# changhaonan/A3VLM

Hardware: AMD Instinct MI355X
Metric: image-text samples/sec (train) + articulation-decode tok/s (higher is better)
Workload: dtype bf16

## Files before the change

### a3vlm_amd/csrc/a3v_train.hip

```cpp
#include "a3v_common.h"

namespace {

template <typename T>
__global__ __launch_bounds__(256) void transpose_kernel(const T* __restrict__ src, int64_t lds_, int64_t bs_s,
                                                        T* __restrict__ dst, int64_t ldd, int64_t bs_d, int R, int C, int Rpad) {
  __shared__ T tile[64][64 + 2];
  const T* s = src + blockIdx.z * bs_s;
  T* d = dst + blockIdx.z * bs_d;
  const int r0 = blockIdx.y * 64, c0 = blockIdx.x * 64;
  const int tx = threadIdx.x & 63, ty = threadIdx.x >> 6;
  for (int i = ty; i < 64; i += 4) {
    const int r = r0 + i, c = c0 + tx;
    tile[i][tx] = (r < R && c < C) ? s[(int64_t)r * lds_ + c] : (T)0.f;
  }
  __syncthreads();
  for (int i = ty; i < 64; i += 4) {
    const int c = c0 + i, r = r0 + tx;
    if (c < C && r < Rpad) d[(int64_t)c * ldd + r] = tile[tx][i];
  }
}

__global__ __launch_bounds__(256) void transpose_bf16_vec_kernel(const bf16_t* __restrict__ src, int64_t lds_, int64_t bs_s,
                                                                 bf16_t* __restrict__ dst, int64_t ldd, int64_t bs_d, int R, int C, int Rpad,
// ... 1125 lines not shown
    if (t.d2) reinterpret_cast<bf16_t*>(t.d2)[r * t.s2r + c * t.s2c] = f2bf(pp);
  }
}
}

extern "C" int a3v_adamw_multi(const a3v_adamw_tensor* table_dev, int n_tensors, int64_t max_n, float lr, float beta1, float beta2, float eps,
                               float weight_decay, int64_t step, const float* grad_scale, void* stream) {
  if (!table_dev || n_tensors <= 0 || max_n <= 0 || step < 1) return A3V_ERR_ARG;
  if (n_tensors > 65535) return A3V_ERR_SHAPE;
  const double bc1 = 1.0 - pow((double)beta1, (double)step), bc2 = 1.0 - pow((double)beta2, (double)step);
  const float step_size = (float)((double)lr / bc1), inv_bc2_sqrt = (float)(1.0 / sqrt(bc2));
  const float decay = (float)(1.0 - (double)lr * (double)weight_decay);
  int64_t blocks = (max_n / 4 + 255) / 256;
  if (blocks > 64) blocks = 64;
  if (blocks < 1) blocks = 1;
  hipLaunchKernelGGL(adamw_multi_kernel, dim3((unsigned)blocks, (unsigned)n_tensors), dim3(256), 0, (hipStream_t)stream, table_dev, decay, beta1,
                     beta2, step_size, inv_bc2_sqrt, eps, grad_scale);
  A3V_LAUNCH_CHECK();
  return A3V_OK;
}

namespace {
__global__ __launch_bounds__(256) void lora_refresh_kernel(const float* __restrict__ wa, const float* __restrict__ wb, int r, int in_f, int nj,
                                                           bf16_t* __restrict__ A, int64_t lda, bf16_t* __restrict__ At, int64_t ldat,
                                                           bf16_t* __restrict__ B, int64_t ldb, bf16_t* __restrict__ Bt, int64_t ldbt,
                                                           int col0, int row0) {
  const int t = blockIdx.x * 256 + threadIdx.x;
  if (t < in_f) {
    for (int i = 0; i < r; ++i) {
      const bf16_t v = f2bf(wa[(int64_t)i * in_f + t]);
      A[(int64_t)(col0 + i) * lda + t] = v;
      At[(int64_t)t * ldat + col0 + i] = v;
    }
  }
  if (t < nj) {
    for (int i = 0; i < r; ++i) {
      const bf16_t v = f2bf(wb[(int64_t)t * r + i]);
      B[(int64_t)(row0 + t) * ldb + col0 + i] = v;
      Bt[(int64_t)(col0 + i) * ldbt + row0 + t] = v;
    }
  }
}
}

extern "C" int a3v_lora_refresh(const float* lora_a, const float* lora_b, int r, int in_f, int nj, void* A, int64_t lda, void* At,
                                int64_t ldat, void* B, int64_t ldb, void* Bt, int64_t ldbt, int col0, int row0, void* stream) {
  if (!lora_a || !lora_b || !A || !At || !B || !Bt || r <= 0 || in_f <= 0 || nj <= 0 || col0 < 0 || row0 < 0) return A3V_ERR_ARG;
  const int n = in_f > nj ? in_f : nj;
  hipLaunchKernelGGL(lora_refresh_kernel, dim3((n + 255) / 256), dim3(256), 0, ST, lora_a, lora_b, r, in_f, nj, (bf16_t*)A, lda, (bf16_t*)At, ldat,
                     (bf16_t*)B, ldb, (bf16_t*)Bt, ldbt, col0, row0);
  A3V_LAUNCH_CHECK();
  return A3V_OK;
}
```

### a3vlm_amd/lib.py

```python
from __future__ import annotations

import ctypes
import os
from ctypes import c_float, c_int, c_int64, c_void_p

_HERE = os.path.dirname(os.path.abspath(__file__))
LIB_PATH = os.environ.get("A3V_LIB_PATH") or os.path.join(_HERE, "liba3vlm_hip.so")

BF16, F32 = 0, 1
EPI_NONE, EPI_BIAS, EPI_GELU, EPI_QUICKGELU, EPI_RESIDUAL, EPI_SWIGLU, EPI_OUT_F32, EPI_RES_F32 = 0, 1, 2, 4, 8, 16, 32, 64
EPI_SWIGLU_BWD = 128

EPI_TILE_128, EPI_TILE_256, EPI_TILE_256PP = 1 << 16, 1 << 17, 1 << 18
EPI_TILE_192PP = 1 << 23

P, I, L, F = c_void_p, c_int, c_int64, c_float

SIGNATURES = {
    "a3v_version": (I, []),
    "a3v_reload_env": (I, []),
    "a3v_gemm_nt": (I, [P, L, P, L, P, L, I, I, I, P, P, L, I, I, P]),
    "a3v_gemm_qkv_rope": (I, [P, L, P, L, I, P, L, P, P, P, L, P, L, P, I, I, I, I, I, I, I, I, P]),
    "a3v_gemm_nt_fp8": (I, [P, L, P, P, L, P, P, L, I, I, I, P, P, L, I, P]),
    "a3v_gemm_qkv_rope_fp8": (I, [P, L, P, P, L, P, I, P, L, P, P, P, I, I, I, I, I, I, I, I, P]),
# ... 8 lines not shown
    "a3v_lora_gb_scatter": (I, [P, L, I, I, P, P, P, P]),
    "a3v_adamw_multi": (I, [P, I, L, F, F, F, F, F, L, P, P]),
    "a3v_scale_cast": (I, [P, I, P, I, L, F, P]),
    "a3v_sumsq_partials": (I, [P, L, P, P]),
    "a3v_grad_bucket_allreduce": (I, [P, P, L, P, I, P]),
    "a3v_grad_bucket_reduce_scatter": (I, [P, P, L, P, P, P, I, P]),
    "a3v_param_shard_all_gather": (I, [P, P, P, L, P]),
    "a3v_rccl_comm_count": (I, [P]),
    "a3v_rccl_available": (I, []),
    "a3v_gemm_nn": (I, [P, L, P, L, P, L, I, I, I, P, L, I, P]),
    "a3v_gemm_tn": (I, [P, L, P, L, P, L, I, I, I, P, L, I, P]),
    "a3v_gemm_tn_sumsq": (I, [P, L, P, L, P, L, I, I, I, P, L, I, P, L, P]),
    "a3v_gemm_tn_sumsq_slots": (L, [I, I]),
    "a3v_gemm_set_workspace": (I, [P, L]),
    "a3v_gemm_set_workspace_for": (I, [P, P, L]),
    "a3v_gemm_nt_splitk": (I, [P, L, P, L, P, I, I, I, I, P]),
    "a3v_splitk_reduce": (I, [P, I, I, I, P, L, I, I, P]),
    "a3v_gemm_skinny_split": (I, [I, I, I]),
    "a3v_gemm_skinny_ws_bytes": (L, [I, I, I]),
    "a3v_gemm_skinny_fp8": (I, [P, L, P, L, P, P, L, I, I, I, P, L, I, P, P]),
    "a3v_quantize_nf4_ws_bytes": (L, [I, I]),
    "a3v_quantize_nf4": (I, [P, I, I, P, P, P, P]),
    "a3v_dequantize_nf4": (I, [P, P, P, L, I, I, P]),
    "a3v_gemm_skinny_nf4": (I, [P, L, P, L, P, P, L, I, I, I, P, L, I, P, P]),
    "a3v_gemm_skinny": (I, [P, L, P, L, P, L, I, I, I, P, L, I, P, P]),
    "a3v_rmsnorm": (I, [P, L, P, P, L, I, I, F, I, I, I, P]),
    "a3v_layernorm": (I, [P, L, P, P, P, L, P, I, I, F, I, I, I, P]),
    "a3v_rope_kvcache": (I, [P, L, P, L, P, P, P, I, I, I, I, I, I, I, I, I, P]),
    "a3v_vt_pack": (I, [P, L, P, I, I, I, I, I, I, P]),
    "a3v_attention_scratch_floats": (L, [I, I, I, I]),
    "a3v_attention": (I, [P, P, P, P, I, I, I, I, I, I, ctypes.POINTER(c_int64), I, P, I, P]),
    "a3v_embed_assemble": (I, [P, L, P, P, I, I, I, I, I, I, I, P]),
    "a3v_fill_rows": (I, [P, P, L, P, I, I, I, I, P]),
    "a3v_patch_im2col": (I, [P, P, I, I, I, I, I, I, I, P]),
    "a3v_split_views": (I, [P, P, I, I, I, I, P]),
    "a3v_vit_embed": (I, [P, P, P, P, I, I, I, I, P]),
    "a3v_argmax": (I, [P, L, P, I, I, P]),
    "a3v_sample_top_p": (I, [P, L, I, I, F, F, P, P, P]),
    "a3v_preprocess_image": (I, [P, I, I, I, I, I, P, P, P, I, P, P, I, I, P, P, I, P, P, P]),
    "a3v_preprocess_batch": (I, [P, I, P, I, P, L, P, L, I, P, P, P]),
    "a3v_generate_step": (I, [P, L, P, I, I, P, L, P, L, I, P, P, I, P, P, P, P]),
    "a3v_count_valid": (I, [P, I, P, P]),
    "a3v_cross_entropy": (I, [P, L, P, P, P, L, P, F, I, I, I, P]),
    "a3v_attention_lse": (I, [P, P, P, P, P, I, I, I, I, I, I, ctypes.POINTER(c_int64), I, I, P]),
    "a3v_transpose": (I, [P, L, L, P, L, L, I, I, I, I, I, P]),
    "a3v_rmsnorm_bwd_scratch_floats": (L, [I, I]),
    "a3v_rmsnorm_bwd": (I, [P, L, P, P, L, P, L, P, P, I, I, F, I, P]),
    "a3v_rmsnorm_bwd_cast": (I, [P, L, P, P, L, P, L, P, P, I, I, F, I, P, L, P]),
    "a3v_rmsnorm_bwd_bf16": (I, [P, L, P, P, L, P, L, P, P, I, I, F, P]),
    "a3v_layernorm_bwd_bf16": (I, [P, L, P, P, L, P, P, L, P, P, I, I, F, P]),
    "a3v_embed_bwd_bf16": (I, [P, L, P, P, I, I, I, I, I, P]),
    "a3v_layernorm_bwd": (I, [P, L, P, P, L, P, P, L, P, P, I, I, F, I, P]),
    "a3v_swiglu_fwd": (I, [P, L, P, L, I, I, I, I, P]),
    "a3v_swiglu_bwd": (I, [P, L, P, L, P, L, I, I, I, I, P]),
    "a3v_cast": (I, [P, L, I, P, L, I, I, I, P]),
    "a3v_add2d": (I, [P, L, P, L, I, I, I, P]),
    "a3v_rope_bwd_pack": (I, [P, P, P, P, L, P, I, I, I, I, I, I, I, P]),
    "a3v_attention_bwd": (I, [P, P, L, L, P, L, L, L, P, P, P, P, P, P, P, P, I, I, I, I, I, I, I, P]),
    "a3v_attention_bwd_workspace_bytes": (L, [I, I, I, I, I]),
    "a3v_attention_bwd_mfma": (I, [P, P, L, L, P, L, L, L, P, P, P, P, P, P, P, I, I, I, I, I, I, P]),
    "a3v_embed_bwd": (I, [P, L, P, P, I, I, I, I, I, P]),
    "a3v_rows_sum": (I, [P, L, P, I, I, P, I, P]),
}

class LlamaLayer(ctypes.Structure):
    _fields_ = [(n, c_void_p) for n in ("attn_norm_w", "wqkv", "wo", "ffn_norm_w", "w13", "w2", "k_cache", "vt_cache",
                                        "wqkv_q", "wqkv_s", "wo_q", "wo_s", "w13_q", "w13_s", "w2_q", "w2_s",
                                        "wqkv_n4", "wqkv_n4s", "wo_n4", "wo_n4s", "w13_n4", "w13_n4s", "w2_n4", "w2_n4s")]


class ImageDesc(ctypes.Structure):
    _fields_ = [("src", c_void_p), ("coeffs", c_void_p), ("bounds", c_void_p), ("H", c_int), ("W", c_int), ("side", c_int), ("pad_x", c_int),
                ("pad_y", c_int), ("ksize", c_int)]


SIGNATURES["a3v_llama_decode_step"] = (I, [ctypes.POINTER(LlamaLayer), I, P, P, P, P, P, P, P, P, I, I, I, I, I, I, I, I, F, P])
SIGNATURES["a3v_llama_decode_step_form"] = (I, [I, I, I, I, I, I, I])

_lib = None


def load() -> ctypes.CDLL:
    global _lib
    if _lib is not None:
        return _lib
    if not os.path.isfile(LIB_PATH):
        raise RuntimeError(
            f"{LIB_PATH} not found: the HIP extension is not built. Run "
            "`python -c 'import __graft_entry__ as g; g.build()'` (or `make -C a3vlm_amd/csrc`). "
            "a3vlm_amd has no non-HIP fallback.")
    import torch
    lib = ctypes.CDLL(LIB_PATH)
    for name, (res, args) in SIGNATURES.items():
        fn = getattr(lib, name)
        fn.restype = res
        fn.argtypes = args
    _lib = lib
    return lib


class env:

    def __init__(self, **kw):
        self.kw = {k: str(v) for k, v in kw.items()}
        self.old = {}

# ... 28 lines not shown
```

### a3vlm_amd/ops.py

```python
from __future__ import annotations

import ctypes
from typing import Optional

import torch

from . import lib as _l
from .lib import BF16, F32, EPI_BIAS, EPI_GELU, EPI_QUICKGELU, EPI_RESIDUAL, EPI_SWIGLU, EPI_OUT_F32, EPI_RES_F32, EPI_SWIGLU_BWD

_DT = {torch.bfloat16: BF16, torch.float32: F32}


def dt(t: torch.Tensor) -> int:
    try:
        return _DT[t.dtype]
    except KeyError:
        raise TypeError(f"a3vlm_amd supports bf16/fp32 tensors, got {t.dtype}")


def _p(t: Optional[torch.Tensor]):
    return None if t is None else t.data_ptr()


def _stream() -> int:
# ... 433 lines not shown


_rb_scratch = {}


def rmsnorm_bwd(x, w, dy, dh, dw, eps, dh_lowp=None):
    _dev(x, w, dy, dh, dw, dh_lowp)
    assert w.dtype == torch.float32 and x.dtype == dh.dtype and x.dtype in (torch.float32, torch.bfloat16)
    rows, dim = x.shape
    scratch = None
    if dw is not None:
        need = int(_l.load().a3v_rmsnorm_bwd_scratch_floats(rows, dim))
        scratch = _rb_scratch.get(x.device)
        if scratch is None or scratch.numel() < need:
            scratch = torch.empty(need, dtype=torch.float32, device=x.device)
            _rb_scratch[x.device] = scratch
    if x.dtype == torch.bfloat16:
        assert dh_lowp is None and dy.dtype == torch.bfloat16
        rc = _l.load().a3v_rmsnorm_bwd_bf16(_p(x), x.stride(0), _p(w), _p(dy), dy.stride(0), _p(dh), dh.stride(0), _p(dw), _p(scratch), rows,
                                            dim, eps, _stream())
        _l.check(rc, "a3v_rmsnorm_bwd_bf16")
        return
    if dh_lowp is not None:
        assert dh_lowp.dtype == torch.bfloat16 and dh_lowp.shape == dh.shape
        rc = _l.load().a3v_rmsnorm_bwd_cast(_p(x), x.stride(0), _p(w), _p(dy), dy.stride(0), _p(dh), dh.stride(0), _p(dw), _p(scratch), rows,
                                            dim, eps, dt(dy), _p(dh_lowp), dh_lowp.stride(0), _stream())
        _l.check(rc, "a3v_rmsnorm_bwd_cast")
        return
    rc = _l.load().a3v_rmsnorm_bwd(_p(x), x.stride(0), _p(w), _p(dy), dy.stride(0), _p(dh), dh.stride(0), _p(dw), _p(scratch), rows, dim,
                                   eps, dt(dy), _stream())
    _l.check(rc, "a3v_rmsnorm_bwd")


def layernorm_bwd(x, w, dy, row_map, dx, dw, db, eps=1e-5):
    _dev(x, w, dy, row_map, dx, dw, db)
    rows, dim = x.shape
    if dy.dtype == torch.bfloat16:
        rc = _l.load().a3v_layernorm_bwd_bf16(_p(x), x.stride(0), _p(w), _p(dy), dy.stride(0), _p(row_map), _p(dx), dx.stride(0),
                                              _p(dw), _p(db), rows, dim, eps, _stream())
        _l.check(rc, "a3v_layernorm_bwd_bf16")
        return
    rc = _l.load().a3v_layernorm_bwd(_p(x), x.stride(0), _p(w), _p(dy), dy.stride(0), _p(row_map), _p(dx), dx.stride(0),
                                     _p(dw), _p(db), rows, dim, eps, dt(x), _stream())
    _l.check(rc, "a3v_layernorm_bwd")


def swiglu_fwd(gu, act, F, interleaved: bool):
    _dev(gu, act)
    rc = _l.load().a3v_swiglu_fwd(_p(gu), gu.stride(0), _p(act), act.stride(0), gu.shape[0], F, 1 if interleaved else 0,
                                  dt(gu), _stream())
    _l.check(rc, "a3v_swiglu_fwd")


def swiglu_bwd(gu, dact, dgu, F, interleaved: bool):
    _dev(gu, dact, dgu)
    rc = _l.load().a3v_swiglu_bwd(_p(gu), gu.stride(0), _p(dact), dact.stride(0), _p(dgu), dgu.stride(0), gu.shape[0], F,
                                  1 if interleaved else 0, dt(gu), _stream())
    _l.check(rc, "a3v_swiglu_bwd")


def rope_bwd_pack(dq, dk, dv, dqkv, cos_sin, B, S, H, Hkv, hd, rope_pos0=0):
    _dev(dq, dk, dv, dqkv, cos_sin)
    rc = _l.load().a3v_rope_bwd_pack(_p(dq), _p(dk), _p(dv), _p(dqkv), dqkv.stride(0), _p(cos_sin), B, S, H, Hkv, hd,
                                     rope_pos0, dt(dq), _stream())
    _l.check(rc, "a3v_rope_bwd_pack")


def attention_bwd_workspace_bytes(B, S, H, Hkv, hd) -> int:
    return _l.load().a3v_attention_bwd_workspace_bytes(B, S, H, Hkv, hd)


def attention_bwd(q, k, k_sb, k_sh, v, v_sb, v_ss, v_sh, out, dout, lse, D, dq, dk, dv, B, S, H, Hkv, hd, causal: bool,
                  workspace=None):
    _dev(q, k, v, out, dout, lse, D, dq, dk, dv, workspace)
    rc = _l.load().a3v_attention_bwd(_p(q), _p(k), k_sb, k_sh, _p(v), v_sb, v_ss, v_sh, _p(out), _p(dout), _p(lse), _p(D),
                                     _p(dq), _p(dk), _p(dv), _p(workspace), B, S, H, Hkv, hd, 1 if causal else 0, dt(q), _stream())
    _l.check(rc, "a3v_attention_bwd")


def attention_bwd_packed(q, k, k_sb, k_sh, v, v_sb, v_ss, v_sh, out, dout, lse, D, dqkv, cos_sin, B, S, H, Hkv, hd, causal: bool,
                         rope_pos0: int = 0):
    _dev(q, k, v, out, dout, lse, D, dqkv, cos_sin)
    ld_out = out.stride(-2) if out.dim() == 2 else out.stride(1)
    rc = _l.load().a3v_attention_bwd_packed(_p(q), _p(k), k_sb, k_sh, _p(v), v_sb, v_ss, v_sh, _p(out), ld_out, _p(dout), _p(lse), _p(D),
                                            _p(dqkv), dqkv.stride(0), _p(cos_sin), rope_pos0, B, S, H, Hkv, hd, 1 if causal else 0,
                                            dt(q), _stream())
    _l.check(rc, "a3v_attention_bwd_packed")


def embed_bwd(tokens, dh, dtable, B, T, W, dim):
    _dev(tokens, dh, dtable)
    assert dh.is_contiguous()
    fn = _l.load().a3v_embed_bwd_bf16 if dh.dtype == torch.bfloat16 else _l.load().a3v_embed_bwd
    rc = fn(_p(tokens), tokens.stride(0), _p(dh), _p(dtable), B, T, W, dim, dtable.shape[0], _stream())
    _l.check(rc, "a3v_embed_bwd")


def rows_sum(src, row_idx, n_rows, out):
    _dev(src, row_idx, out)
    rc = _l.load().a3v_rows_sum(_p(src), src.stride(0), _p(row_idx), n_rows, src.shape[1], _p(out), dt(src), _stream())
    _l.check(rc, "a3v_rows_sum")


def lora_gb_scatter(gbt, r: int, views, row0s):
    import ctypes
    _dev(gbt, *views)
# ... 21 lines not shown
```

### a3vlm_amd/train.py

```python
from __future__ import annotations

import os

from typing import Callable, Dict, List, Optional, Tuple

import torch

from . import ops
from .util import install_param_epoch_hook, optimizer_steps, param_state_key


def _pad64(n: int) -> int:
    return (n + 63) // 64 * 64


def skinny_slices(M: int, N: int, K: int, cus: int) -> int:
    blocks = ((M + 127) // 128) * ((N + 127) // 128)
    nk = K // 64
    S = 1
    while blocks * S < 512 and S * 2 <= nk and S < 32:
        S *= 2
    if N <= 64 and M >= 2048 and cus > 0:
        S = max(1, min(cus // ((M + 255) // 256), nk // 2, 32))
    elif N <= 64 and M >= 512 and S > 4:
# ... 427 lines not shown
                    blk.copy_(li[key + ".B"])
                    li[key + ".B"] = blk
                    rows_a = fy[fy.shape[0] - Rp:]
                    rows_a.copy_(li[key + ".A"])
                    li[key + ".A"] = rows_a
                    if self._nt_dgrad(key):
                        ft = im[key + ".yT"]
                        cols_at = ft[:, ft.shape[1] - Rp:]
                        cols_at.copy_(li[key + ".At"][:cols_at.shape[0]])
                        li[key + ".At"] = cols_at
        self._li, self._li_ver, self._li_act = li, ver, self.act
        self._li_checked = True
        self._adapter_sinks = None
        return li

    def adapter_sink(self, p: torch.Tensor):
        li = getattr(self, "_li", None)
        if li is None or self.act != torch.bfloat16 or getattr(self, "_li_act", None) != self.act:
            return None
        sinks = getattr(self, "_adapter_sinks", None)
        if sinks is None:
            sinks = {}
            r = self.m.lora_rank
            for i in range(self.m.n_layers):
                for key, mods, _ in self.m.lora_groups(i):
                    A, Bm, At, Bt = li[key + ".A"], li[key + ".B"], li[key + ".At"], li[key + ".Bt"]
                    row = 0
                    for j, mod in enumerate(mods):
                        wa, wb = mod.lora_a.weight, mod.lora_b.weight
                        sinks[id(wa)] = (A.data_ptr() + 2 * (j * r) * A.stride(0), A.stride(0), 1,
                                         At.data_ptr() + 2 * (j * r), 1, At.stride(0))
                        sinks[id(wb)] = (Bm.data_ptr() + 2 * (row * Bm.stride(0) + j * r), Bm.stride(0), 1,
                                         Bt.data_ptr() + 2 * ((j * r) * Bt.stride(0) + row), 1, Bt.stride(0))
                        row += wb.shape[0]
            self._adapter_sinks = sinks
        return sinks.get(id(p))

    def adapters_adopted(self, written_ids) -> None:
        plist = getattr(self, "_lora_plist", None)
        if plist is None or getattr(self, "_li", None) is None:
            return
        if all(id(q) in written_ids for q in plist if q.requires_grad):
            self._li_ver = tuple(param_state_key(q) for q in plist)

    def _lora_fwd(self, key: str, x: torch.Tensor, y: torch.Tensor, tag: str) -> torch.Tensor:
        li = self._lora_step_images()
        A, Bm = li[key + ".A"], li[key + ".B"]
        t = self._buf("lora_t." + key.split(".")[0] + tag, (x.shape[0], A.shape[0]))
        self._skinny(x, A, t)
        f32 = y.dtype == torch.float32 and self.act == torch.bfloat16
        ops.gemm_nt(t, Bm, y, residual=y, epilogue=ops.EPI_RES_F32 if f32 else 0)
        return t

    def _kx_group_bwd(self, i: int, key: str, dy_full: torch.Tensor, N: int, x: torch.Tensor, t: torch.Tensor, dx: torch.Tensor,
                      swiglu_gu: Optional[torch.Tensor] = None):
        li = self._lora_step_images()
        dy, dt = dy_full[:, :N], dy_full[:, N:]
        self._dgrad(dy, li[key + ".Bt"], dt)
        im = self._images()
        if swiglu_gu is not None:
            ops.gemm_nt(dy_full, im[key + ".yT"], dx, residual=swiglu_gu, epilogue=ops.EPI_SWIGLU_BWD)
        elif self._nt_dgrad(key):
            ops.gemm_nt(dy_full, im[key + ".yT"], dx)
        else:
            ops.gemm_nn(dy_full, im[key + ".y"], dx)
        self._lora_bwd(i, key, dy, x, t, None, dt=dt)

    def _lora_bwd(self, i: int, key: str, dy: torch.Tensor, x: torch.Tensor, t: torch.Tensor, dx: Optional[torch.Tensor], dt=None):
        m = self.m
        li = self._lora_step_images()
        r = m.lora_rank
        Bt, At = li[key + ".Bt"], li[key + ".At"]
        M, N = dy.shape
        Rp = t.shape[1]
        if dt is None:
            dt = self._buf("lora_dt", (M, Rp))
            self._dgrad(dy, Bt, dt)
        g = key.split(".")[0]
        names = {"qkv": ["attention.wq", "attention.wk", "attention.wv"], "wo": ["attention.wo"],
                 "w13": ["feed_forward.w1", "feed_forward.w3"], "w2": ["feed_forward.w2"]}[g]
        vas = [self._views[f"layers.{i}.{nm}.lora_a.weight"] for nm in names]
        vbs = [self._views[f"layers.{i}.{nm}.lora_b.weight"] for nm in names]
        nr = len(names) * r
        gBt = self._buf("lora_gBt." + g, (Rp, N), torch.float32)
        self._wgrad(t, dy, gBt, "lb", store=True)
        adjacent = all(vas[j + 1].data_ptr() == vas[j].data_ptr() + 4 * vas[j].numel() for j in range(len(vas) - 1))
        if adjacent and dt.stride(0) % 8 == 0:
            off = (vas[0].data_ptr() - self._flat.data_ptr()) // 4
            self._wgrad(dt[:, :nr], x, self._flat[off:off + nr * x.shape[1]].view(nr, x.shape[1]), "la", store=False)
        else:
            gA = self._buf("lora_gA." + g, (Rp, x.shape[1]), torch.float32)
            self._wgrad(dt, x, gA, "la", store=True)
            for j, va in enumerate(vas):
                ops.add2d(va, gA[j * r:(j + 1) * r])
        row0s, row = [], 0
        for vb in vbs:
            row0s.append(row)
            row += vb.shape[0]
        if gBt.is_cuda:
            ops.lora_gb_scatter(gBt, r, vbs, row0s)
        else:
            for j, vb in enumerate(vbs):
                vb.add_(gBt[j * r:(j + 1) * r, row0s[j]:row0s[j] + vb.shape[0]].t())
        if dx is not None:
            ops.gemm_nt(dt, At, dx, residual=dx)

    def _block_forward(self, i: int, h: torch.Tensor, B: int, S: int, keep: bool, tag: str = "", h_out: Optional[torch.Tensor] = None):
        m, a, im = self.m, self.m.args, self._images()
        H, Hkv, hd, dim, F = m.n_heads, m.n_kv_heads, m.head_dim, a.dim, m.ffn
        rows = B * S
        l = m.layers[i]
        spad = _pad64(S)
        kx = self._kext() > 0 and rows > 16 and hd in (64, 128) and self.fuse_qkv_rope
        li = self._lora_step_images() if kx else None

        def xbuf(name, cols, key):
            ext = li[key + ".A"].shape[0]
            full = self._buf(name + tag, (rows, cols + ext))
            return full, full[:, :cols], full[:, cols:]
        if kx:
            xn_full, xn, t_qkv = xbuf("xn", dim, f"qkv.{i}")
            att_full, att, t_wo = xbuf("att", H * hd, f"wo.{i}")
        else:
            xn = self._buf("xn" + tag, (rows, dim))
            att = self._buf("att" + tag, (rows, H * hd))
        qkv = self._buf("qkv" + tag, (rows, (H + 2 * Hkv) * hd))
        qrot = self._buf("qrot" + tag, (rows, H * hd))
        kc = self._buf("kc" + tag, (B, Hkv, spad, hd))
        vc = self._buf("vc", (B, Hkv, hd, spad))
        lse = self._buf("lse" + tag, (B, H, S), torch.float32)
        ops.rmsnorm(h, l.attention_norm.weight, xn, a.norm_eps)
        lt = {}
        if not self.lora and self.act == torch.bfloat16 and hd in (64, 128) and rows > 16 and self.fuse_qkv_rope:
            ops.gemm_qkv_rope(xn, im[f"qkv.{i}"], qrot, kc, vc, m._cos_sin_dev(), B, S, H, Hkv, hd, 0, 0,
                              v_rows=qkv[:, (H + Hkv) * hd:])
        elif kx:
            self._skinny(xn, li[f"qkv.{i}.A"], t_qkv)
            ops.gemm_qkv_rope(xn_full, im[f"qkv.{i}.x"], qrot, kc, vc, m._cos_sin_dev(), B, S, H, Hkv, hd, 0, 0,
                              v_rows=qkv[:, (H + Hkv) * hd:])
            lt["qkv"] = t_qkv
        elif self.lora and self.act == torch.bfloat16 and hd in (64, 128) and rows > 16 and self.fuse_qkv_rope:
            li = self._lora_step_images()
            A, Bm = li[f"qkv.{i}.A"], li[f"qkv.{i}.B"]
            t = self._buf("lora_t.qkv" + tag, (rows, A.shape[0]))
            self._skinny(xn, A, t)
            ops.gemm_nt(t, Bm, qkv)
            ops.gemm_qkv_rope(xn, im[f"qkv.{i}"], qrot, kc, vc, m._cos_sin_dev(), B, S, H, Hkv, hd, 0, 0,
                              v_rows=qkv[:, (H + Hkv) * hd:], delta=qkv)
            lt["qkv"] = t
        else:
            ops.gemm_nt(xn, im[f"qkv.{i}"], qkv)
            if self.lora:
                lt["qkv"] = self._lora_fwd(f"qkv.{i}", xn, qkv, tag)
            ops.rope_kvcache(qkv, qrot, kc, vc, m._cos_sin_dev(), B, S, H, Hkv, hd, 0, 0)
        ldo = att.stride(0)
        strides = (S * H * hd, H * hd, hd, Hkv * spad * hd, spad * hd, hd, Hkv * hd * spad, hd * spad, spad, S * ldo, ldo, hd)
        ops.attention_lse(qrot, kc, vc, att, lse, B, S, S, H, Hkv, hd, strides, True)
        res_flag = ops.EPI_RES_F32 if (self.act == torch.bfloat16 and self.stream == torch.float32) else 0
        h_mid = self._buf("h_mid" + tag, (rows, dim), self.stream) if keep else h
        if kx:
            self._skinny(att, li[f"wo.{i}.A"], t_wo)
            ops.gemm_nt(att_full, im[f"wo.{i}.x"], h_mid, residual=h, epilogue=res_flag)
            lt["wo"] = t_wo
        else:
            ops.gemm_nt(att, im[f"wo.{i}"], h_mid, residual=h, epilogue=res_flag)
            if self.lora:
                lt["wo"] = self._lora_fwd(f"wo.{i}", att, h_mid, tag)
        gu = self._buf("gu" + tag, (rows, 2 * F))
        if kx:
            xn2_full, xn2, t_w13 = xbuf("xn2", dim, f"w13.{i}")
            act_full, actb, t_w2 = xbuf("act", F, f"w2.{i}")
        else:
            xn2 = self._buf("xn2" + tag, (rows, dim))
            actb = self._buf("act" + tag, (rows, F))
        ops.rmsnorm(h_mid, l.ffn_norm.weight, xn2, a.norm_eps)
        if kx:
            self._skinny(xn2, li[f"w13.{i}.A"], t_w13)
            ops.gemm_nt(xn2_full, im[f"w13.{i}.x"], gu)
            lt["w13"] = t_w13
        else:
            ops.gemm_nt(xn2, im[f"w13.{i}"], gu)
            if self.lora:
                lt["w13"] = self._lora_fwd(f"w13.{i}", xn2, gu, tag)
        ops.swiglu_fwd(gu, actb, F, interleaved=False)
        if kx:
            self._skinny(actb, li[f"w2.{i}.A"], t_w2)
            lt["w2"] = t_w2
        elif self.lora:
            li2 = self._lora_step_images()
            lt["w2"] = self._buf("lora_t.w2" + tag, (rows, li2[f"w2.{i}.A"].shape[0]))
            self._skinny(actb, li2[f"w2.{i}.A"], lt["w2"])
        kept = dict(xn=xn, qkv=qkv, qrot=qrot, kc=kc, att=att, lse=lse, h_mid=h_mid, xn2=xn2, gu=gu, act=actb, spad=spad, lt=lt)
        if keep and h_out is None:
            return kept
        out = h_out if keep else h
        if kx:
            ops.gemm_nt(act_full, im[f"w2.{i}.x"], out, residual=h_mid, epilogue=res_flag)
            return kept
        ops.gemm_nt(actb, im[f"w2.{i}"], out, residual=h_mid, epilogue=res_flag)
        if self.lora:
            f32 = out.dtype == torch.float32 and self.act == torch.bfloat16
            ops.gemm_nt(lt["w2"], self._lora_step_images()[f"w2.{i}.B"], out, residual=out, epilogue=ops.EPI_RES_F32 if f32 else 0)
        return kept

    def _block_backward(self, i: int, h_in: torch.Tensor, dh: torch.Tensor, B: int, S: int):
        m, a, im = self.m, self.m.args, self._images()
        H, Hkv, hd, dim, F = m.n_heads, m.n_kv_heads, m.head_dim, a.dim, m.ffn
        rows = B * S
        l = m.layers[i]
        pre = f"layers.{i}."
        k = self._saved["kept"][i] if self._saved.get("kept") else self._block_forward(i, h_in, B, S, keep=True)
        lt = k.get("lt", {})
        kx = self._kext() > 0 and rows > 16 and hd in (64, 128) and self.fuse_qkv_rope
        li = self._lora_step_images() if kx else None

        def ybuf(name, cols, key):
            full = self._buf(name, (rows, cols + li[key + ".A"].shape[0]))
            return full, full[:, :cols]
        stream_lp = self.stream == torch.bfloat16 and self.act == torch.bfloat16
        if stream_lp:
            dha = dh
            dha_full = self._dh_full if kx else None
        elif kx:
            dha_full, dha = ybuf("dh_act.x", dim, f"w2.{i}")
        else:
            dha = self._buf("dh_act", (rows, dim))
        fuse_cast = self.act == torch.bfloat16 and not stream_lp
        if not stream_lp and not (fuse_cast and getattr(self, "_dha_ready", False)):
            ops.cast(dh, dha)
        self._dha_ready = False
        if self._has(pre + "feed_forward.w2.weight"):
            self._wgrad(dha, k["act"], self._views[pre + "feed_forward.w2.weight"], "w2", (pre + "feed_forward.w2.weight",))
        if kx and self.fuse_swiglu_bwd and self._nt_dgrad(f"w2.{i}") and F % 8 == 0:
            dgu_full, dgu = ybuf("dgu.x", 2 * F, f"w13.{i}")
            self._kx_group_bwd(i, f"w2.{i}", dha_full, dim, k["act"], lt["w2"], dgu, swiglu_gu=k["gu"])
        elif (not self.lora and self.fuse_swiglu_bwd and self.nn_dgrad and self.act == torch.bfloat16 and dim % 64 == 0 and F % 8 == 0 and F >= 256
              and dha.stride(0) % 8 == 0 and 2 * rows * dha.stride(0) < 2 ** 31 and 2 * F * dim < 2 ** 31
              and tuple(im[f"w2.{i}"].shape) == (dim, F)):
            dgu = self._buf("dgu", (rows, 2 * F))
# ... 482 lines not shown
```

### include/a3vlm_hip.h

```cpp
#ifndef A3VLM_HIP_H
#define A3VLM_HIP_H

#include <stdint.h>

#ifdef __cplusplus
extern "C" {
#endif

enum { A3V_BF16 = 0, A3V_F32 = 1 };

enum {
  A3V_OK = 0,
  A3V_ERR_SHAPE = -1,
  A3V_ERR_DTYPE = -2,
  A3V_ERR_ARG = -3
};

enum {
  A3V_EPI_NONE = 0,
  A3V_EPI_BIAS = 1,
  A3V_EPI_GELU = 2,
  A3V_EPI_QUICKGELU = 4,
  A3V_EPI_RESIDUAL = 8,
  A3V_EPI_SWIGLU = 16,
// ... 129 lines not shown
  const void* wo;
  const void* ffn_norm_w;
  const void* w13;
  const void* w2;
  void* k_cache;
  void* vt_cache;
  const void* wqkv_q; const float* wqkv_s;
  const void* wo_q;   const float* wo_s;
  const void* w13_q;  const float* w13_s;
  const void* w2_q;   const float* w2_s;
  const void* wqkv_n4; const float* wqkv_n4s;
  const void* wo_n4;   const float* wo_n4s;
  const void* w13_n4;  const float* w13_n4s;
  const void* w2_n4;   const float* w2_n4s;
} a3v_llama_layer;
int a3v_llama_decode_step(const a3v_llama_layer* layers, int n_layers, void* h, void* xn, void* qkv,
                          void* att, void* act, float* attn_scratch, void* skinny_ws, const float* cos_sin, int B,
                          int dim, int H, int Hkv, int hd, int ffn, int Smax, int pos, float eps,
                          void* stream);
int a3v_llama_decode_step_form(int B, int dim, int H, int Hkv, int hd, int ffn, int w8);


int a3v_attention_lse(const void* q, const void* k, const void* vt, void* out, float* lse, int B,
                      int Sq, int Sk, int H, int Hkv, int hd, const int64_t* strides, int causal,
                      int dtype, void* stream);

int a3v_transpose(const void* src, int64_t ld_src, int64_t bs_src, void* dst, int64_t ld_dst,
                  int64_t bs_dst, int R, int C, int Rpad, int batch, int dtype, void* stream);

int64_t a3v_rmsnorm_bwd_scratch_floats(int rows, int dim);
int a3v_rmsnorm_bwd(const float* x, int64_t ldx, const float* w, const void* dy, int64_t lddy,
                    float* dh, int64_t lddh, float* dw, float* dw_scratch, int rows, int dim, float eps,
                    int act_dtype, void* stream);
int a3v_rmsnorm_bwd_cast(const float* x, int64_t ldx, const float* w, const void* dy, int64_t lddy,
                         float* dh, int64_t lddh, float* dw, float* dw_scratch, int rows, int dim, float eps,
                         int act_dtype, void* dh_bf16, int64_t ld_bf16, void* stream);

int a3v_rmsnorm_bwd_bf16(const void* x, int64_t ldx, const float* w, const void* dy, int64_t lddy, void* dh, int64_t lddh,
                         float* dw, float* dw_scratch, int rows, int dim, float eps, void* stream);
int a3v_layernorm_bwd_bf16(const void* x, int64_t ldx, const float* w, const void* dy, int64_t lddy, const int32_t* row_map,
                           void* dx, int64_t lddx, float* dw, float* db, int rows, int dim, float eps, void* stream);
int a3v_embed_bwd_bf16(const int64_t* tokens, int64_t ld_tok, const void* dh, float* dtable, int B, int T, int W, int dim,
                       int vocab, void* stream);

int a3v_layernorm_bwd(const void* x, int64_t ldx, const float* w, const float* dy, int64_t lddy,
                      const int32_t* row_map, void* dx, int64_t lddx, float* dw, float* db, int rows,
                      int dim, float eps, int act_dtype, void* stream);

int a3v_swiglu_fwd(const void* gu, int64_t ldg, void* act, int64_t lda, int rows, int F,
                   int interleaved, int dtype, void* stream);
int a3v_swiglu_bwd(const void* gu, int64_t ldg, const void* dact, int64_t lda, void* dgu,
                   int64_t lddg, int rows, int F, int interleaved, int dtype, void* stream);

int a3v_rope_bwd_pack(const void* dq, const void* dk, const void* dv, void* dqkv, int64_t ld,
                      const float* cos_sin, int B, int S, int H, int Hkv, int hd, int rope_pos0,
                      int dtype, void* stream);

int a3v_attention_bwd(const void* q, const void* k, int64_t k_sb, int64_t k_sh, const void* v,
                      int64_t v_sb, int64_t v_ss, int64_t v_sh, const void* out, const void* dout,
                      const float* lse, float* D, void* dq, void* dk, void* dv, void* workspace,
                      int B, int S, int H, int Hkv, int hd, int causal, int dtype, void* stream);
int a3v_attention_bwd_packed(const void* q, const void* k, int64_t k_sb, int64_t k_sh, const void* v, int64_t v_sb,
                             int64_t v_ss, int64_t v_sh, const void* out, int64_t ld_out, const void* dout, const float* lse, float* D,
                             void* dqkv, int64_t ld_qkv, const float* cos_sin, int rope_pos0, int B, int S, int H, int Hkv,
                             int hd, int causal, int dtype, void* stream);
int64_t a3v_attention_bwd_workspace_bytes(int B, int S, int H, int Hkv, int hd);
int a3v_attention_bwd_mfma(const void* q, const void* k, int64_t k_sb, int64_t k_sh, const void* v,
                           int64_t v_sb, int64_t v_ss, int64_t v_sh, const void* dout, const float* lse,
                           const float* D, void* dq, void* dk, void* dv, void* workspace, int B, int S,
                           int H, int Hkv, int hd, int causal, void* stream);

int a3v_add2d(void* dst, int64_t ld_dst, const void* src, int64_t ld_src, int rows, int cols, int dtype, void* stream);
int a3v_cast(const void* src, int64_t ld_src, int src_dtype, void* dst, int64_t ld_dst, int dst_dtype,
             int rows, int cols, void* stream);

int a3v_embed_bwd(const int64_t* tokens, int64_t ld_tok, const float* dh, float* dtable, int B, int T,
                  int W, int dim, int vocab, void* stream);

int a3v_rows_sum(const void* src, int64_t ld, const int32_t* row_idx, int n_rows, int dim, float* out,
                 int dtype, void* stream);

int a3v_adamw(float* param, const float* grad, float* exp_avg, float* exp_avg_sq, int64_t n, float lr, float beta1, float beta2,
              float eps, float weight_decay, int64_t step, void* bf16_image, void* stream);

int a3v_adamw_scaled(float* param, const float* grad, float* exp_avg, float* exp_avg_sq, int64_t n, float lr, float beta1, float beta2,
                     float eps, float weight_decay, int64_t step, void* bf16_image, const float* grad_scale, void* stream);

int a3v_lora_gb_scatter(const float* gbt, int64_t ld, int r, int n_mods, float* const* dst, const int* row0, const int* nj, void* stream);

int a3v_gemm_tn_strip(const void* T, int64_t ldt, const void* X, int64_t ldx, float* partial, int R, int N, int Kt, int S, void* stream);

int a3v_adamw_scaled_t(float* param, const float* grad, float* exp_avg, float* exp_avg_sq, int rows, int cols, float lr, float beta1,
                       float beta2, float eps, float weight_decay, int64_t step, void* bf16_image, void* bf16_image_t, int64_t ldt,
                       const float* grad_scale, void* stream);

typedef struct {
  float* p; const float* g; float* m; float* v;
  int64_t n, cols;
  void* d1; int64_t s1r, s1c;
  void* d2; int64_t s2r, s2c;
} a3v_adamw_tensor;
int a3v_adamw_multi(const a3v_adamw_tensor* table, int n_tensors, int64_t max_n, float lr, float beta1, float beta2, float eps,
                    float weight_decay, int64_t step, const float* grad_scale, void* stream);

int a3v_scale_cast(const void* src, int src_dtype, void* dst, int dst_dtype, int64_t n, float scale, void* stream);

// ... 19 lines not shown
```

Baseline: 35.87.

## Fuse RMSNorm and SwiGLU with the LoRA down-projection skinny GEMM

```diff
diff --git a/a3vlm_amd/csrc/a3v_train.hip b/a3vlm_amd/csrc/a3v_train.hip
--- a/a3vlm_amd/csrc/a3v_train.hip
+++ b/a3vlm_amd/csrc/a3v_train.hip
@@ -1201,3 +1201,203 @@
   A3V_LAUNCH_CHECK();
   return A3V_OK;
 }
+
+
+constexpr int RP_ROWS = 16;
+constexpr int RP_N = 64;
+
+__device__ __forceinline__ void rowproj_load_w(const bf16_t* __restrict__ W, int64_t ldw, int r, int k, bf16x8 (&wf)[2][4]) {
+#pragma unroll
+  for (int j = 0; j < 4; ++j) {
+    const bf16_t* p = W + (int64_t)(j * 16 + r) * ldw + k;
+    wf[0][j] = *reinterpret_cast<const bf16x8*>(p);
+    wf[1][j] = *reinterpret_cast<const bf16x8*>(p + 8);
+  }
+}
+__device__ __forceinline__ void rowproj_mma(f32x4 (&acc)[4], const bf16x8 (&wf)[4], bf16x8 xf) {
+#pragma unroll
+  for (int j = 0; j < 4; ++j) acc[j] = __builtin_amdgcn_mfma_f32_16x16x32_bf16(wf[j], xf, acc[j], 0, 0, 0);
+}
+__device__ __forceinline__ void rowproj_finish(const f32x4 (&acc)[4], float* part, bf16_t* __restrict__ t, int64_t ldt, int row0, int rows) {
+  const int wv = threadIdx.x >> 6, lane = threadIdx.x & 63;
+#pragma unroll
+  for (int j = 0; j < 4; ++j)
+#pragma unroll
+    for (int i = 0; i < 4; ++i) part[(wv * 16 + j * 4 + i) * 64 + lane] = acc[j][i];
+  __syncthreads();
+  const int row = row0 + (lane & 15);
+  bf16x4 o;
+#pragma unroll
+  for (int i = 0; i < 4; ++i) {
+    float s = part[(wv * 4 + i) * 64 + lane];
+#pragma unroll
+    for (int w = 1; w < 4; ++w) s += part[(w * 16 + wv * 4 + i) * 64 + lane];
+    o[i] = (bf16_t)s;
+  }
+  if (row < rows) *reinterpret_cast<bf16x4*>(t + (int64_t)row * ldt + wv * 16 + (lane >> 4) * 4) = o;
+}
+
+namespace {
+template <int NT>
+__global__ __launch_bounds__(256) void swiglu_fwd_proj_kernel(const bf16_t* __restrict__ gu, int64_t ldg, bf16_t* __restrict__ act, int64_t lda,
+                                                              const bf16_t* __restrict__ W, int64_t ldw, bf16_t* __restrict__ t, int64_t ldt,
+                                                              int rows, int F) {
+  __shared__ float part[4 * 16 * 64];
+  const int wv = threadIdx.x >> 6, lane = threadIdx.x & 63, r = lane & 15, g = lane >> 4;
+  const int row0 = blockIdx.x * RP_ROWS, row = row0 + r;
+  const bool live = row < rows;
+  const int nslab = F >> 6;
+  const bf16_t* gr = gu + (int64_t)(live ? row : row0) * ldg + g * 16;
+  bf16_t* ar = act + (int64_t)row * lda + g * 16;
+  f32x4 acc[4];
+#pragma unroll
+  for (int j = 0; j < 4; ++j) acc[j] = f32x4{0.f, 0.f, 0.f, 0.f};
+  bf16x8 gv[2], uv[2], wf[2][4];
+  auto load = [&](int s, bf16x8 (&gq)[2], bf16x8 (&uq)[2], bf16x8 (&wq)[2][4]) {
+    const bf16x8* p = reinterpret_cast<const bf16x8*>(gr + s * 64);
+    const bf16x8* q = reinterpret_cast<const bf16x8*>(gr + F + s * 64);
+#pragma unroll
+    for (int h = 0; h < 2; ++h) {
+      gq[h] = (NT & 1) ? __builtin_nontemporal_load(p + h) : p[h];
+      uq[h] = (NT & 1) ? __builtin_nontemporal_load(q + h) : q[h];
+    }
+    rowproj_load_w(W, ldw, r, s * 64 + g * 16, wq);
+  };
+  if (wv < nslab) load(wv, gv, uv, wf);
+  for (int s = wv; s < nslab; s += 4) {
+    bf16x8 gn[2], un[2], wn[2][4];
+    load(s + 4 < nslab ? s + 4 : s, gn, un, wn);
+#pragma unroll
+    for (int h = 0; h < 2; ++h) {
+      bf16x8 o;
+#pragma unroll
+      for (int e = 0; e < 8; ++e) {
+        const float gf = (float)gv[h][e], uf = (float)uv[h][e];
+        o[e] = (bf16_t)(rbf(gf * __builtin_amdgcn_rcpf(1.f + __expf(-gf))) * uf);
+      }
+      if (live) {
+        bf16x8* d = reinterpret_cast<bf16x8*>(ar + s * 64 + h * 8);
+        if (NT & 2) __builtin_nontemporal_store(o, d); else *d = o;
+      }
+      rowproj_mma(acc, wf[h], o);
+    }
+#pragma unroll
+    for (int h = 0; h < 2; ++h) {
+      gv[h] = gn[h]; uv[h] = un[h];
+#pragma unroll
+      for (int j = 0; j < 4; ++j) wf[h][j] = wn[h][j];
+    }
+  }
+  rowproj_finish(acc, part, t, ldt, row0, rows);
+}
+
+template <typename TW, int MAXS>
+__global__ __launch_bounds__(256, MAXS <= 16 ? 2 : 1) void rmsnorm_proj_kernel(const bf16_t* __restrict__ x, int64_t ldx, const TW* __restrict__ w,
+                                                           bf16_t* __restrict__ y, int64_t ldy, const bf16_t* __restrict__ W, int64_t ldw,
+                                                           bf16_t* __restrict__ t, int64_t ldt, int rows, int dim, float eps) {
+  __shared__ float part[4 * 16 * 64];
+  __shared__ float red[4][16];
+  const int wv = threadIdx.x >> 6, lane = threadIdx.x & 63, r = lane & 15, g = lane >> 4;
+  const int row0 = blockIdx.x * RP_ROWS, row = row0 + r;
+  const bool live = row < rows;
+  const int nslab = dim >> 6;
+  const bf16_t* xr = x + (int64_t)(live ? row : row0) * ldx + g * 16;
+  bf16_t* yr = y + (int64_t)row * ldy + g * 16;
+  bf16x8 xv[MAXS][2];
+  float ss = 0.f;
+#pragma unroll
+  for (int i = 0; i < MAXS; ++i) {
+    const int s = wv + 4 * i;
+    const bool on = live && s < nslab;
+#pragma unroll
+    for (int h = 0; h < 2; ++h) {
+      bf16x8 z;
+#pragma unroll
+      for (int e = 0; e < 8; ++e) z[e] = (bf16_t)0.f;
+      xv[i][h] = on ? *reinterpret_cast<const bf16x8*>(xr + s * 64 + h * 8) : z;
+    }
+  }
+#pragma unroll
+  for (int i = 0; i < MAXS; ++i)
+#pragma unroll
+    for (int h = 0; h < 2; ++h)
+#pragma unroll
+      for (int e = 0; e < 8; ++e) { const float v = (float)xv[i][h][e]; ss = fmaf(v, v, ss); }
+  {
+    float a, b;
+    lane_xchg32(ss, a, b); ss = a + b;
+    lane_xchg16(ss, a, b); ss = a + b;
+  }
+  if (g == 0) red[wv][r] = ss;
+  __syncthreads();
+#pragma unroll
+  for (int i = 0; i < MAXS; ++i)
+#pragma unroll
+    for (int h = 0; h < 2; ++h) {
+      u32x4 q = __builtin_bit_cast(u32x4, xv[i][h]);
+      asm volatile("" : "+v"(q));
+      xv[i][h] = __builtin_bit_cast(bf16x8, q);
+    }
+  ss = ((red[0][r] + red[1][r]) + red[2][r]) + red[3][r];
+  const float inv = rsqrtf(ss / (float)dim + eps);
+  f32x4 acc[4];
+#pragma unroll
+  for (int j = 0; j < 4; ++j) acc[j] = f32x4{0.f, 0.f, 0.f, 0.f};
+  bf16x8 wf[2][2][4];
+  rowproj_load_w(W, ldw, r, wv * 64 + g * 16, wf[0]);
+#pragma unroll
+  for (int i = 0; i < MAXS; ++i) {
+    const int s = wv + 4 * i;
+    const int k = (s < nslab ? s : wv) * 64 + g * 16;
+    if (i + 1 < MAXS) {
+      const int sn = s + 4;
+      rowproj_load_w(W, ldw, r, (sn < nslab ? sn : wv) * 64 + g * 16, wf[(i + 1) & 1]);
+    }
+#pragma unroll
+    for (int h = 0; h < 2; ++h) {
+      float wn[8];
+      load8(w + k + h * 8, wn);
+      bf16x8 o;
+#pragma unroll
+      for (int e = 0; e < 8; ++e) o[e] = (bf16_t)(rbf((float)xv[i][h][e] * inv) * wn[e]);
+      if (live && s < nslab) *reinterpret_cast<bf16x8*>(yr + s * 64 + h * 8) = o;
+      rowproj_mma(acc, wf[i & 1][h], o);
+    }
+    __builtin_amdgcn_sched_barrier(0);
+  }
+  rowproj_finish(acc, part, t, ldt, row0, rows);
+}
+}
+
+static bool rowproj_args_ok(const void* W, int64_t ldw, const void* t, int64_t ldt, int K) {
+  return W && t && K >= 256 && K % 64 == 0 && ldw >= K && ldw % 8 == 0 && ldt >= RP_N && ldt % 4 == 0 && ((uintptr_t)W & 15) == 0 &&
+         ((uintptr_t)t & 7) == 0;
+}
+
+extern "C" int a3v_swiglu_fwd_proj(const void* gu, int64_t ldg, void* act, int64_t lda, const void* W, int64_t ldw, void* t, int64_t ldt,
+                                   int rows, int F, void* stream) {
+  if (!gu || !act || rows <= 0 || F <= 0) return A3V_ERR_ARG;
+  if (!rowproj_args_ok(W, ldw, t, ldt, F) || ldg < 2 * (int64_t)F || lda < F || (ldg % 8) || (lda % 8) || (((uintptr_t)gu | (uintptr_t)act) & 15))
+    return A3V_ERR_SHAPE;
+  hipLaunchKernelGGL((swiglu_fwd_proj_kernel<STREAM_NT>), dim3((rows + RP_ROWS - 1) / RP_ROWS), dim3(256), 0, ST, (const bf16_t*)gu, ldg,
+                     (bf16_t*)act, lda, (const bf16_t*)W, ldw, (bf16_t*)t, ldt, rows, F);
+  A3V_LAUNCH_CHECK();
+  return A3V_OK;
+}
+
+extern "C" int a3v_rmsnorm_proj(const void* x, int64_t ldx, const void* w, void* y, int64_t ldy, const void* W, int64_t ldw, void* t,
+                                int64_t ldt, int rows, int dim, float eps, int w_dtype, void* stream) {
+  if (!x || !w || !y || rows <= 0 || dim <= 0) return A3V_ERR_ARG;
+  if (!rowproj_args_ok(W, ldw, t, ldt, dim) || dim > 5120 || ldx < dim || ldy < dim || (ldx % 8) || (ldy % 8) ||
+      (((uintptr_t)x | (uintptr_t)y | (uintptr_t)w) & 15))
+    return A3V_ERR_SHAPE;
+  if (w_dtype != A3V_BF16 && w_dtype != A3V_F32) return A3V_ERR_DTYPE;
+  const dim3 grid((rows + RP_ROWS - 1) / RP_ROWS), blk(256);
+#define A3V_RP(TW, MS) hipLaunchKernelGGL((rmsnorm_proj_kernel<TW, MS>), grid, blk, 0, ST, (const bf16_t*)x, ldx, (const TW*)w, (bf16_t*)y, ldy, \
+                                          (const bf16_t*)W, ldw, (bf16_t*)t, ldt, rows, dim, eps)
+  if (w_dtype == A3V_BF16) { if (dim <= 4096) A3V_RP(bf16_t, 16); else A3V_RP(bf16_t, 20); }
+  else { if (dim <= 4096) A3V_RP(float, 16); else A3V_RP(float, 20); }
+#undef A3V_RP
+  A3V_LAUNCH_CHECK();
+  return A3V_OK;
+}
diff --git a/a3vlm_amd/lib.py b/a3vlm_amd/lib.py
--- a/a3vlm_amd/lib.py
+++ b/a3vlm_amd/lib.py
@@ -84,6 +84,8 @@
     "a3v_embed_bwd_bf16": (I, [P, L, P, P, I, I, I, I, I, P]),
     "a3v_layernorm_bwd": (I, [P, L, P, P, L, P, P, L, P, P, I, I, F, I, P]),
     "a3v_swiglu_fwd": (I, [P, L, P, L, I, I, I, I, P]),
+    "a3v_swiglu_fwd_proj": (I, [P, L, P, L, P, L, P, L, I, I, P]),
+    "a3v_rmsnorm_proj": (I, [P, L, P, P, L, P, L, P, L, I, I, F, I, P]),
     "a3v_swiglu_bwd": (I, [P, L, P, L, P, L, I, I, I, I, P]),
     "a3v_cast": (I, [P, L, I, P, L, I, I, I, P]),
     "a3v_add2d": (I, [P, L, P, L, I, I, I, P]),
diff --git a/a3vlm_amd/ops.py b/a3vlm_amd/ops.py
--- a/a3vlm_amd/ops.py
+++ b/a3vlm_amd/ops.py
@@ -509,6 +509,31 @@
     _l.check(rc, "a3v_swiglu_fwd")
 
 
+def row_proj_ok(x, W, t) -> bool:
+    K = W.shape[1]
+    return (x.is_cuda and x.dtype == W.dtype == t.dtype == torch.bfloat16 and W.shape[0] == 64 and t.shape[1] == 64 and K % 64 == 0
+            and K >= 256 and W.stride(1) == 1 and W.stride(0) % 8 == 0 and t.stride(1) == 1 and t.stride(0) % 4 == 0
+            and W.data_ptr() % 16 == 0 and t.data_ptr() % 8 == 0)
+
+
+def swiglu_fwd_proj(gu, act, F, W, t):
+    _dev(gu, act, W, t)
+    assert row_proj_ok(act, W, t) and W.shape[1] == F and gu.dtype == torch.bfloat16
+    rc = _l.load().a3v_swiglu_fwd_proj(_p(gu), gu.stride(0), _p(act), act.stride(0), _p(W), W.stride(0), _p(t), t.stride(0),
+                                       gu.shape[0], F, _stream())
+    _l.check(rc, "a3v_swiglu_fwd_proj")
+
+
+def rmsnorm_proj(x, w, out, eps: float, W, t):
+    _dev(x, w, out, W, t)
+    rows, dim = x.shape
+    assert row_proj_ok(out, W, t) and W.shape[1] == dim and x.dtype == torch.bfloat16
+    rc = _l.load().a3v_rmsnorm_proj(_p(x), x.stride(0), _p(w), _p(out), out.stride(0), _p(W), W.stride(0), _p(t), t.stride(0),
+                                    rows, dim, eps, dt(w), _stream())
+    _l.check(rc, "a3v_rmsnorm_proj")
+    return out
+
+
 def swiglu_bwd(gu, dact, dgu, F, interleaved: bool):
     _dev(gu, dact, dgu)
     rc = _l.load().a3v_swiglu_bwd(_p(gu), gu.stride(0), _p(dact), dact.stride(0), _p(dgu), dgu.stride(0), gu.shape[0], F,
diff --git a/a3vlm_amd/train.py b/a3vlm_amd/train.py
--- a/a3vlm_amd/train.py
+++ b/a3vlm_amd/train.py
@@ -503,6 +503,13 @@
         ops.gemm_nt(t, Bm, y, residual=y, epilogue=ops.EPI_RES_F32 if f32 else 0)
         return t
 
+    def _norm_proj(self, h: torch.Tensor, w: torch.Tensor, xn: torch.Tensor, A: torch.Tensor, t: torch.Tensor) -> bool:
+        dim = h.shape[1]
+        if not (h.dtype == torch.bfloat16 and dim <= 5120 and h.stride(0) % 8 == 0 and xn.stride(0) % 8 == 0 and ops.row_proj_ok(xn, A, t)):
+            return False
+        ops.rmsnorm_proj(h, w, xn, self.m.args.norm_eps, A, t)
+        return True
+
     def _kx_group_bwd(self, i: int, key: str, dy_full: torch.Tensor, N: int, x: torch.Tensor, t: torch.Tensor, dx: torch.Tensor,
                       swiglu_gu: Optional[torch.Tensor] = None):
         li = self._lora_step_images()
@@ -580,13 +587,16 @@
         kc = self._buf("kc" + tag, (B, Hkv, spad, hd))
         vc = self._buf("vc", (B, Hkv, hd, spad))
         lse = self._buf("lse" + tag, (B, H, S), torch.float32)
-        ops.rmsnorm(h, l.attention_norm.weight, xn, a.norm_eps)
+        qkv_t_done = kx and self._norm_proj(h, l.attention_norm.weight, xn, li[f"qkv.{i}.A"], t_qkv)
+        if not qkv_t_done:
+            ops.rmsnorm(h, l.attention_norm.weight, xn, a.norm_eps)
         lt = {}
         if not self.lora and self.act == torch.bfloat16 and hd in (64, 128) and rows > 16 and self.fuse_qkv_rope:
             ops.gemm_qkv_rope(xn, im[f"qkv.{i}"], qrot, kc, vc, m._cos_sin_dev(), B, S, H, Hkv, hd, 0, 0,
                               v_rows=qkv[:, (H + Hkv) * hd:])
         elif kx:
-            self._skinny(xn, li[f"qkv.{i}.A"], t_qkv)
+            if not qkv_t_done:
+                self._skinny(xn, li[f"qkv.{i}.A"], t_qkv)
             ops.gemm_qkv_rope(xn_full, im[f"qkv.{i}.x"], qrot, kc, vc, m._cos_sin_dev(), B, S, H, Hkv, hd, 0, 0,
                               v_rows=qkv[:, (H + Hkv) * hd:])
             lt["qkv"] = t_qkv
@@ -624,18 +634,25 @@
         else:
             xn2 = self._buf("xn2" + tag, (rows, dim))
             actb = self._buf("act" + tag, (rows, F))
-        ops.rmsnorm(h_mid, l.ffn_norm.weight, xn2, a.norm_eps)
         if kx:
-            self._skinny(xn2, li[f"w13.{i}.A"], t_w13)
+            if not self._norm_proj(h_mid, l.ffn_norm.weight, xn2, li[f"w13.{i}.A"], t_w13):
+                ops.rmsnorm(h_mid, l.ffn_norm.weight, xn2, a.norm_eps)
+                self._skinny(xn2, li[f"w13.{i}.A"], t_w13)
             ops.gemm_nt(xn2_full, im[f"w13.{i}.x"], gu)
             lt["w13"] = t_w13
         else:
+            ops.rmsnorm(h_mid, l.ffn_norm.weight, xn2, a.norm_eps)
             ops.gemm_nt(xn2, im[f"w13.{i}"], gu)
             if self.lora:
                 lt["w13"] = self._lora_fwd(f"w13.{i}", xn2, gu, tag)
-        ops.swiglu_fwd(gu, actb, F, interleaved=False)
+        w2_t_done = kx and ops.row_proj_ok(actb, li[f"w2.{i}.A"], t_w2)
+        if w2_t_done:
+            ops.swiglu_fwd_proj(gu, actb, F, li[f"w2.{i}.A"], t_w2)
+        else:
+            ops.swiglu_fwd(gu, actb, F, interleaved=False)
         if kx:
-            self._skinny(actb, li[f"w2.{i}.A"], t_w2)
+            if not w2_t_done:
+                self._skinny(actb, li[f"w2.{i}.A"], t_w2)
             lt["w2"] = t_w2
         elif self.lora:
             li2 = self._lora_step_images()
diff --git a/include/a3vlm_hip.h b/include/a3vlm_hip.h
--- a/include/a3vlm_hip.h
+++ b/include/a3vlm_hip.h
@@ -205,6 +205,11 @@
 int a3v_swiglu_bwd(const void* gu, int64_t ldg, const void* dact, int64_t lda, void* dgu,
                    int64_t lddg, int rows, int F, int interleaved, int dtype, void* stream);
 
+int a3v_swiglu_fwd_proj(const void* gu, int64_t ldg, void* act, int64_t lda, const void* W, int64_t ldw,
+                        void* t, int64_t ldt, int rows, int F, void* stream);
+int a3v_rmsnorm_proj(const void* x, int64_t ldx, const void* w, void* y, int64_t ldy, const void* W,
+                     int64_t ldw, void* t, int64_t ldt, int rows, int dim, float eps, int w_dtype, void* stream);
+
 int a3v_rope_bwd_pack(const void* dq, const void* dk, const void* dv, void* dqkv, int64_t ld,
                       const float* cos_sin, int B, int S, int H, int Hkv, int hd, int rope_pos0,
                       int dtype, void* stream);
```

Result: slower. 35.27 (-1.7%).
